# fboehm/DBSLMM

Measured on AMD Instinct MI355X. Metric: SNPs solved/sec (whole node) + max-|Δβ| vs CPU ref, 1M SNP × 10k indiv, higher is better.
Workload: dtype f64

## Files before the change

### dbslmm_amd/csrc/pcg.hip

```cpp
#include <hip/hip_runtime.h>
#include <stdint.h>

namespace pcg {
constexpr int kT = 128;
constexpr int kRunMax = 8;
constexpr int kMaxNC = 4;
constexpr int kWaves = 4;
constexpr int kVS = kT + 8;
constexpr int kNDot = 5;
constexpr int kQS = 8;
constexpr int kThreads = 256;
constexpr int kFTb = 8;
constexpr int kFRows = kFTb * kT;
constexpr int kFPer = kFRows / kThreads;
__device__ __forceinline__ void chip_wide_priority() { __builtin_amdgcn_s_setprio(3); }
constexpr int wave_lds_doubles(int nc) { return 3 * nc * kVS + 4 * nc * 64; }
constexpr size_t lds_bytes(int nc) { return sizeof(double) * kWaves * wave_lds_doubles(nc); }
}

struct PcgBlk {
    int32_t blk, row0, m, ms;
    int32_t ld, Tb, Ns, sco;
    int64_t matoff, vo, po, dof;
    int64_t off16;
    int32_t nc;
    int32_t mshift;
    int32_t fused;
    int32_t pad_;
};

struct PcgArgs {
    const PcgBlk* blk;
    const uint16_t* G16;
    const double* M;
    const int32_t* flags;
    const double* S;
    const double* rsd;
    const double* z;
    const int32_t* slot_out;
    const int32_t* blk_id;
    const double* dshift;
    double *X, *R, *P, *Sv, *W;
    double* U;
    double* part;
    double* dot;
    double* qs;
    int32_t* cnv;
    int32_t* itb;
    int32_t* done;
    int32_t* active;
    int32_t* fin;
    double* beta_s;
    double* beta_l;
    int32_t* status;
    double* mir_s;
    double* mir_l;
    int32_t* mir_st;
    int32_t* mir_flag;
    int32_t run_no;
    int64_t vstride;
    int64_t ns, nl, nbk;
    double tau, rn, c0, tol, inv_sqrt_n;
    int32_t ncopy;
    int32_t run;
    int32_t seed;
};

namespace pcg {

__device__ __forceinline__ void wave_fence() {
    __builtin_amdgcn_fence(__ATOMIC_RELEASE, "wavefront");
    __builtin_amdgcn_wave_barrier();
    __builtin_amdgcn_fence(__ATOMIC_ACQUIRE, "wavefront");
}

template <int Ctrl>
__device__ __forceinline__ double dpp_mov(double v) {
    const uint64_t b = __builtin_bit_cast(uint64_t, v);
    const int lo = __builtin_amdgcn_mov_dpp(static_cast<int>(b & 0xffffffffu), Ctrl, 0xf, 0xf, false);
    const int hi = __builtin_amdgcn_mov_dpp(static_cast<int>(b >> 32), Ctrl, 0xf, 0xf, false);
    return __builtin_bit_cast(double, (static_cast<uint64_t>(static_cast<uint32_t>(hi)) << 32) | static_cast<uint32_t>(lo));
}
template <int X>
__device__ __forceinline__ uint32_t swap_xor(uint32_t x, bool up) {
    if constexpr (X == 16) {
        const auto r = __builtin_amdgcn_permlane16_swap(x, x, false, false);
        return up ? r[0] : r[1];
    } else {
        const auto r = __builtin_amdgcn_permlane32_swap(x, x, false, false);
        return up ? r[0] : r[1];
    }
}
template <int X>
__device__ __forceinline__ double lane_xor(double v) {
#ifndef PCG_NO_DPP
    if constexpr (X == 1) return dpp_mov<0xB1>(v);
    else if constexpr (X == 2) return dpp_mov<0x4E>(v);
    else if constexpr (X == 4) return dpp_mov<0x1B>(dpp_mov<0x141>(v));
    else if constexpr (X == 8) return dpp_mov<0x128>(v);
#ifndef PCG_NO_PERMLANE
    else if constexpr (X == 16 || X == 32) {
        const uint64_t b = __builtin_bit_cast(uint64_t, v);
        const bool up = (__lane_id() & X) != 0;
        const uint32_t lo = swap_xor<X>(static_cast<uint32_t>(b & 0xffffffffu), up);
        const uint32_t hi = swap_xor<X>(static_cast<uint32_t>(b >> 32), up);
        return __builtin_bit_cast(double, (static_cast<uint64_t>(hi) << 32) | lo);
    }
#endif
    else
#endif
        return __shfl_xor(v, X);
}

template <int X2, int X1, int X0>
__device__ __forceinline__ double rscatter8(const double (&v)[8], int lane) {
    const bool h2 = (lane & X2) != 0, h1 = (lane & X1) != 0, h0 = (lane & X0) != 0;
    double u[4], w[2];
#pragma unroll
    for (int q = 0; q < 4; ++q) {
        const double send = h2 ? v[q] : v[q + 4], keep = h2 ? v[q + 4] : v[q];
        u[q] = keep + lane_xor<X2>(send);
    }
#pragma unroll
    for (int q = 0; q < 2; ++q) {
        const double send = h1 ? u[q] : u[q + 2], keep = h1 ? u[q + 2] : u[q];
        w[q] = keep + lane_xor<X1>(send);
    }
    const double send = h0 ? w[0] : w[1], keep = h0 ? w[1] : w[0];
    return keep + lane_xor<X0>(send);
}

__device__ __forceinline__ double wave_sum(double v) {
    v += lane_xor<32>(v);
    v += lane_xor<16>(v);
    v += lane_xor<8>(v);
    v += lane_xor<4>(v);
    v += lane_xor<2>(v);
    v += lane_xor<1>(v);
    return v;
}



__device__ __forceinline__ double ordered_sum(const double* __restrict__ p, int64_t st, int s0, int s1, double acc) {
    for (int s = s0; s < s1; s += 8) {
        double t[8];
#pragma unroll
        for (int u = 0; u < 8; ++u) t[u] = s + u < s1 ? p[static_cast<int64_t>(s + u) * st] : 0.0;
#pragma unroll
        for (int u = 0; u < 8; ++u) acc += t[u];
    }
    return acc;
}

__device__ __forceinline__ bool on_u16(const PcgArgs& a, const PcgBlk& B) {
    return a.G16 != nullptr && (a.flags[B.blk] & 1) == 0;
}

__device__ __forceinline__ double jdiag(const PcgArgs& a, const PcgBlk& B, int i, double dc) {
    return B.mshift ? 1.0 : i < B.ms ? a.c0 + dc : a.c0;
}
__device__ __forceinline__ double col_shift(const PcgArgs& a, const PcgBlk& B, int k) {
    return a.dshift[B.mshift ? a.seed : k];
}

__device__ __forceinline__ void put_beta(const PcgArgs& a, const PcgBlk& B, int i, int k, double x, bool mono) {
    const int so = a.slot_out[B.row0 + i];
    const double bv = mono ? __builtin_nan("") : x * a.inv_sqrt_n;
    if (so >= 0) {
        a.beta_s[k * a.ns + so] = bv;
        if (a.mir_s) a.mir_s[k * a.ns + so] = bv;
    } else {
        a.beta_l[k * a.nl - 1 - so] = bv;
        if (a.mir_l) a.mir_l[k * a.nl - 1 - so] = bv;
    }
}
__device__ __forceinline__ void put_status(const PcgArgs& a, const PcgBlk& B, int k, bool mono) {
    const int st = mono ? DBSLMM_BLOCK_MONOMORPHIC
                        : a.cnv[B.sco + k] == 0 ? DBSLMM_BLOCK_NOT_CONVERGED : DBSLMM_BLOCK_OK;
    const int64_t o = k * a.nbk + a.blk_id[B.blk];
    a.status[o] = st;
    if (a.mir_st) a.mir_st[o] = st;
}

__device__ __forceinline__ double cvt_lo(uint32_t w) {
    double g;
    uint32_t t;
    asm volatile("v_and_b32 %1, 0xffff, %2\n\tv_cvt_f64_u32 %0, %1" : "=v"(g), "=&v"(t) : "v"(w));
    return g;
}
__device__ __forceinline__ double cvt_hi(uint32_t w) {
    double g;
    uint32_t t;
    asm volatile("v_lshrrev_b32 %1, 16, %2\n\tv_cvt_f64_u32 %0, %1" : "=v"(g), "=&v"(t) : "v"(w));
    return g;
}

typedef uint32_t pcg_u4 __attribute__((ext_vector_type(4)));

__device__ __forceinline__ void cvt_row(const pcg_u4& w, double (&g)[8]) {
#pragma unroll
    for (int c = 0; c < 8; ++c) g[c] = (c & 1) ? cvt_hi(w[c >> 1]) : cvt_lo(w[c >> 1]);
}

__device__ __forceinline__ __amdgpu_buffer_rsrc_t g16_rsrc(const uint16_t* base, uint32_t bytes) {
    const uint64_t gb = reinterpret_cast<uint64_t>(base);
    const uint32_t lo = static_cast<uint32_t>(__builtin_amdgcn_readfirstlane(static_cast<int>(gb & 0xffffffffu)));
    const uint32_t hi = static_cast<uint32_t>(__builtin_amdgcn_readfirstlane(static_cast<int>(gb >> 32)));
    const int nb = __builtin_amdgcn_readfirstlane(static_cast<int>(bytes));
    return __builtin_amdgcn_make_buffer_rsrc(reinterpret_cast<void*>((static_cast<uint64_t>(hi) << 32) | lo),
                                             static_cast<short>(0), nb, 0x00020000);
}
constexpr uint32_t kG16Oob = 0x80000000u;

__device__ __forceinline__ void quad_mul16(const pcg_u4 (&raw)[8], bool diagq, int lane, int nc,
                                           const double* vI, const double* vJ, double* rsum, double* csum) {
    const int rg = lane >> 3, cg = lane & 7;
#pragma unroll 1
    for (int k = 0; k < nc; ++k) {
        double vi[8], vj[8], racc[8], cacc[8];
#pragma unroll
        for (int q = 0; q < 8; ++q) {
            vi[q] = vI[k * kVS + 8 * rg + q];
            vj[q] = vJ[k * kVS + 8 * cg + q];
            racc[q] = cacc[q] = 0.0;
        }
        if (!diagq) {
#pragma unroll
            for (int r = 0; r < 8; ++r) {
                double g[8];
                cvt_row(raw[r], g);
#pragma unroll
                for (int c = 0; c < 8; ++c) {
                    racc[r] = __builtin_fma(g[c], vj[c], racc[r]);
                    cacc[c] = __builtin_fma(g[c], vi[r], cacc[c]);
                }
            }
        } else {
#pragma unroll
            for (int r = 0; r < 8; ++r) {
                double g[8];
                cvt_row(raw[r], g);
#pragma unroll
                for (int c = 0; c < 8; ++c) {
                    const int dd = 8 * (cg - rg) + c - r;
                    racc[r] = __builtin_fma(dd <= 0 ? g[c] : 0.0, vj[c], racc[r]);
                    cacc[c] = __builtin_fma(dd < 0 ? g[c] : 0.0, vi[r], cacc[c]);
                }
            }
        }
        rsum[k * 64 + lane] += rscatter8<4, 2, 1>(racc, lane);
        csum[k * 64 + lane] += rscatter8<32, 16, 8>(cacc, lane);
    }
}

__device__ __forceinline__ void quad_mul64(const double* __restrict__ base, int64_t ld, int rows_ok, int cols_ok,
                                           bool diagq, int lane, int nc, const double* vI, const double* vJ,
                                           double* rsum, double* csum) {
    const int rg = lane >> 3, cg = lane & 7;
#pragma unroll 1
    for (int k = 0; k < nc; ++k) {
        double vi[8], vj[8], racc[8], cacc[8];
#pragma unroll
        for (int q = 0; q < 8; ++q) {
            vi[q] = vI[k * kVS + 8 * rg + q];
            vj[q] = vJ[k * kVS + 8 * cg + q];
            racc[q] = cacc[q] = 0.0;
        }
#pragma unroll 1
        for (int r = 0; r < 8; ++r)
#pragma unroll
            for (int c = 0; c < 8; ++c) {
                const double g = (r < rows_ok && c < cols_ok) ? base[r * ld + c] : 0.0;
                const int dd = 8 * (cg - rg) + c - r;
                const double gr = !diagq || dd <= 0 ? g : 0.0, gc = !diagq || dd < 0 ? g : 0.0;
#pragma unroll
                for (int q = 0; q < 8; ++q)
                    if (q == r) racc[q] = __builtin_fma(gr, vj[c], racc[q]);
                cacc[c] = __builtin_fma(gc, vi[r], cacc[c]);
            }
        rsum[k * 64 + lane] += rscatter8<4, 2, 1>(racc, lane);
        csum[k * 64 + lane] += rscatter8<32, 16, 8>(cacc, lane);
    }
}

__device__ __forceinline__ void stage_v(const PcgArgs& a, const PcgBlk& B, int T, int nc, int lane, double* v) {
    for (int k = 0; k < nc; ++k) {
        const double* src = a.U + k * a.vstride + B.vo + static_cast<int64_t>(T) * kT;
        const double x0 = src[lane], x1 = src[lane + 64];
        v[k * kVS + lane] = x0;
        v[k * kVS + lane + 64] = x1;
    }
}

__device__ __forceinline__ bool quad_active(const PcgBlk& B, int I, int J, int q) {
    const int qi = q >> 1, qj = q & 1;
    return !(J == I && qj > qi) && I * kT + 64 * qi < B.m && J * kT + 64 * qj < B.m;
}
__device__ __forceinline__ bool next_quad(const PcgBlk& B, int I, int J1, int& J, int& q) {
    for (;;) {
        if (++q == 4) {
            q = 0;
            if (++J > J1) return false;
        }
        if (quad_active(B, I, J, q)) return true;
    }
}

template <bool U16>
__device__ void symv_item(const PcgArgs& a, int4 item, int lane, double* vI, double* vJb, double* rsum,
                          double* csum) {
    const PcgBlk B = a.blk[item.x];
    if (a.done[item.x] || on_u16(a, B) != U16) return;
    const int I = item.y, J0 = item.z, J1 = item.w, nc = B.nc;
    const int64_t ld16 = static_cast<int64_t>(B.Tb) * kT;
    const int rg = lane >> 3, cg = lane & 7;
    auto vj_of = [&](int J) -> double* { return J == I ? vI : vJb + ((J - J0) & 1) * nc * kVS; };
    const __amdgpu_buffer_rsrc_t g16 =
        g16_rsrc(a.G16 + B.off16 + static_cast<int64_t>(I) * kT * ld16, U16 ? static_cast<uint32_t>(kT * ld16 * 2) : 0u);
    auto load = [&](int J, int q, pcg_u4 (&raw)[8], bool none) {
        if constexpr (U16) {
            const int i0 = 64 * (q >> 1) + 8 * rg, j0 = J * kT + 64 * (q & 1) + 8 * cg;
            const bool skip = none || j0 >= B.m || (J == I && (q == 0 || q == 3) && cg > rg);
            const uint32_t o = static_cast<uint32_t>((static_cast<int64_t>(i0) * ld16 + j0) * 2);
#pragma unroll
            for (int r = 0; r < 8; ++r)
                raw[r] = __builtin_amdgcn_raw_buffer_load_b128(
                    g16, (skip || I * kT + i0 + r >= B.m) ? kG16Oob : o + static_cast<uint32_t>(r * ld16 * 2), 0, 0);
        }
    };
    auto mult = [&](int J, int q, const pcg_u4 (&raw)[8]) {
        const int qi = q >> 1, qj = q & 1;
        const bool dq = J == I && qi == qj;
        const double* vj = vj_of(J);
        double* rs = rsum + qi * nc * 64;
        double* cs = csum + qj * nc * 64;
        if constexpr (U16) {
            quad_mul16(raw, dq, lane, nc, vI + 64 * qi, vj + 64 * qj, rs, cs);
        } else {
            const int ib = I * kT + 64 * qi + 8 * rg, jb = J * kT + 64 * qj + 8 * cg;
            quad_mul64(a.M + B.matoff + static_cast<int64_t>(ib) * B.ld + jb, B.ld, B.m - ib, B.m - jb, dq,
                       lane, nc, vI + 64 * qi, vj + 64 * qj, rs, cs);
        }
    };
    auto flush = [&](int J) {
        double* dst = a.part + B.po + (static_cast<int64_t>(J) * B.Ns + I) * nc * kT;
        for (int qj = 0; qj < 2; ++qj)
            for (int k = 0; k < nc; ++k) {
                dst[k * kT + 64 * qj + 8 * cg + rg] = csum[(qj * nc + k) * 64 + lane];
                csum[(qj * nc + k) * 64 + lane] = 0.0;
            }
    };
    pcg_u4 ra[8], rb[8];
    int J = J0, q = 0;
    load(J, q, ra, false);
    stage_v(a, B, I, nc, lane, vI);
    if (J != I) stage_v(a, B, J, nc, lane, vj_of(J));
    for (int t = 0; t < 2 * nc; ++t) rsum[t * 64 + lane] = csum[t * 64 + lane] = 0.0;
    wave_fence();
    auto step = [&](pcg_u4 (&cur)[8], pcg_u4 (&nxt)[8]) -> bool {
        int Jn = J, qn = q;
        const bool more = next_quad(B, I, J1, Jn, qn);
        load(more ? Jn : J, more ? qn : q, nxt, !more);
        if (more && Jn != J && Jn != I) stage_v(a, B, Jn, nc, lane, vj_of(Jn));
        mult(J, q, cur);
        if (!more || Jn != J) flush(J);
        wave_fence();
        J = Jn;
        q = qn;
        return more;
    };
    while (step(ra, rb) && step(rb, ra)) {
    }
    double* dst = a.part + B.po + (static_cast<int64_t>(I) * B.Ns + B.Tb + J0 / a.run) * nc * kT;
    for (int qi = 0; qi < 2; ++qi)
        for (int k = 0; k < nc; ++k) dst[k * kT + 64 * qi + 8 * rg + cg] = rsum[(qi * nc + k) * 64 + lane];
}

}

extern "C" __global__ __launch_bounds__(pcg::kThreads) void dbslmm_pcg_init(PcgArgs a, const int2* __restrict__ rows,
                                                                            int32_t n_lead, int32_t skip) {
    using namespace pcg;
    __shared__ double red[kThreads / 64][kMaxNC];
    __shared__ int mono_s;
    const int g = blockIdx.x;
    const int2 it = rows[g < n_lead ? g : g + skip];
    const bool head = it.y < 0;
    const int bi = it.x, I = head ? 0 : it.y, tid = threadIdx.x;
    const PcgBlk B = a.blk[bi];
    const bool u16 = on_u16(a, B);
    const int n = a.ncopy, nc = B.nc;
    if (I == 0) {
        if (tid == 0) mono_s = 0;
        __syncthreads();
        bool mono = false;
        for (int i = tid; i < B.m; i += kThreads) mono |= !(a.rsd[B.row0 + i] < INFINITY);
        if (mono) atomicOr(&mono_s, 1);
        __syncthreads();
        if (tid < n) {
            a.cnv[B.sco + tid] = 0;
            double* q = a.qs + static_cast<int64_t>(B.sco + tid) * kQS;
            q[4] = q[5] = 1.0;
        }
        if (tid == 0) {
            a.itb[bi] = 0;
            a.fin[bi] = 0;
            const bool fz = B.fused && u16;
            a.done[bi] = mono_s ? 2 : fz ? 3 : 0;
            if (!mono_s && !fz) atomicAdd(a.active, 1);
        }
    }
    if (head) return;
    const int r = tid & (kT - 1), h = tid >> 7, i = I * kT + r;
    const bool in = i < B.m;
    double sv[kMaxNC];
#pragma unroll
    for (int k = 0; k < kMaxNC; ++k) sv[k] = 0.0;
    for (int c = h; c < n; c += 2) {
        const int64_t o = c * a.vstride + B.vo + i;
        const double rhs = in ? a.z[B.row0 + i] : 0.0;
        a.X[o] = 0.0;
        a.P[o] = 0.0;
        if (c < nc) {
            a.Sv[o] = 0.0;
            a.W[o] = 0.0;
            a.R[o] = rhs;
            double uv = 0.0;
            if (in) {
                uv = rhs / jdiag(a, B, i, col_shift(a, B, c));
                if (u16) uv *= a.rsd[B.row0 + i];
            }
            a.U[o] = uv;
        }
    }
#pragma unroll
    for (int k = 0; k < kMaxNC; ++k)
        if (k < nc && (k & 1) == h && in && u16) {
            const double rhs = a.z[B.row0 + i];
            sv[k] = a.S[B.row0 + i] * a.rsd[B.row0 + i] * (rhs / jdiag(a, B, i, col_shift(a, B, k)));
        }
#pragma unroll
    for (int k = 0; k < kMaxNC; ++k) sv[k] = wave_sum(sv[k]);
    if ((tid & 63) == 0)
#pragma unroll
        for (int k = 0; k < kMaxNC; ++k) red[tid >> 6][k] = sv[k];
    __syncthreads();
    if (tid < nc) {
        const int hk = tid & 1;
        a.dot[B.dof + (static_cast<int64_t>(I) * kNDot + 4) * n + tid] = red[2 * hk][tid] + red[2 * hk + 1][tid];
    }
}

template <bool U16>
__device__ __forceinline__ void symv_body(const PcgArgs& a, const int4* __restrict__ items, int32_t n_items) {
    using namespace pcg;
    extern __shared__ double vlds[];
    chip_wide_priority();
    const int wave = threadIdx.x >> 6, lane = threadIdx.x & 63;
    const int e = blockIdx.x * kWaves + wave;
    if (e >= n_items) return;
    const int nc = a.ncopy;
    double* w = vlds + wave * wave_lds_doubles(nc);
    symv_item<U16>(a, items[e], lane, w, w + nc * kVS, w + 3 * nc * kVS, w + 3 * nc * kVS + 2 * nc * 64);
}
#ifndef PCG_SYMV_WAVES
#define PCG_SYMV_WAVES 2
#endif
extern "C" __global__ __launch_bounds__(pcg::kThreads) __attribute__((amdgpu_waves_per_eu(PCG_SYMV_WAVES, 8)))
void dbslmm_pcg_symv16(PcgArgs a, const int4* __restrict__ items, int32_t n_items) {
    symv_body<true>(a, items, n_items);
}
extern "C" __global__ __launch_bounds__(pcg::kThreads)
void dbslmm_pcg_symv64(PcgArgs a, const int4* __restrict__ items, int32_t n_items) {
    symv_body<false>(a, items, n_items);
}

extern "C" __global__ __launch_bounds__(pcg::kThreads) void dbslmm_pcg_rows(PcgArgs a, const int2* __restrict__ rows) {
    using namespace pcg;
    __shared__ double red[kThreads / 64][kMaxNC][4];
    __shared__ double sig[kMaxNC];
    chip_wide_priority();
    const int2 it = rows[blockIdx.x];
    const int bi = it.x, I = it.y, tid = threadIdx.x;
    if (a.done[bi]) return;
    const PcgBlk B = a.blk[bi];
    const bool u16 = on_u16(a, B);
    const int n = a.ncopy, nc = B.nc;
    if (tid < nc)
        sig[tid] = ordered_sum(a.dot + B.dof + 4 * n + tid, kNDot * n, 0, B.Tb, 0.0);
    __syncthreads();
    const int r = tid & (kT - 1), h = tid >> 7, i = I * kT + r;
    const bool in = i < B.m;
    const double Si = in ? a.S[B.row0 + i] : 0.0, ri = in ? a.rsd[B.row0 + i] : 0.0;
    const int nrun = (I + a.run) / a.run;
    double dv[kMaxNC][4];
#pragma unroll
    for (int k = 0; k < kMaxNC; ++k)
#pragma unroll
        for (int f = 0; f < 4; ++f) dv[k][f] = 0.0;
#pragma unroll
    for (int k = 0; k < kMaxNC; ++k) {
        if (k >= n || (k & 1) != h) continue;
        const int64_t o = k * a.vstride + B.vo + i;
        if (k < nc) {
            const double* pp = a.part + B.po + static_cast<int64_t>(I) * B.Ns * nc * kT + k * kT + r;
            double y = ordered_sum(pp, nc * kT, I, B.Tb, 0.0);
            y = ordered_sum(pp, nc * kT, B.Tb, B.Tb + nrun, y);
            const double dc = col_shift(a, B, k);
            const double rv = a.R[o];
            const double u = in ? rv / jdiag(a, B, i, dc) : 0.0;
            const double sh = i < B.ms ? dc : 0.0;
            double w = 0.0;
            if (in) {
                if (u16) w = a.tau * a.rn * ri * __builtin_fma(-Si, sig[k] * a.rn, y) + (1.0 - a.tau + sh) * u;
                else w = y + sh * u;
            }
            a.W[o] = w;
            dv[k][0] = rv * u;
            dv[k][1] = w * u;
            dv[k][2] = rv * rv;
        }
        const double xv = a.X[o];
        dv[k][3] = xv * xv;
    }
#pragma unroll
    for (int k = 0; k < kMaxNC; ++k)
#pragma unroll
        for (int f = 0; f < 4; ++f) dv[k][f] = wave_sum(dv[k][f]);
    if ((tid & 63) == 0)
#pragma unroll
        for (int k = 0; k < kMaxNC; ++k)
#pragma unroll
            for (int f = 0; f < 4; ++f) red[tid >> 6][k][f] = dv[k][f];
    __syncthreads();
    if (tid < 4 * n) {
        const int k = tid >> 2, f = tid & 3, hk = k & 1;
        if (f == 3 || k < nc)
            a.dot[B.dof + (static_cast<int64_t>(I) * kNDot + f) * n + k] = red[2 * hk][k][f] + red[2 * hk + 1][k][f];
    }
    if (I == 0 && tid == 0) a.itb[bi] += 1;
}

extern "C" __global__ __launch_bounds__(pcg::kThreads) void dbslmm_pcg_update(PcgArgs a, const int2* __restrict__ rows) {
    using namespace pcg;
    __shared__ double tot[kMaxNC][4];
    __shared__ double coef[kMaxNC][3];
    __shared__ double seedc[2];
    __shared__ int run_s[kMaxNC];
    __shared__ double red[kThreads / 64][kMaxNC];
    chip_wide_priority();
    const int2 it = rows[blockIdx.x];
    const int bi = it.x, I = it.y, tid = threadIdx.x;
    if (a.done[bi]) return;
    const PcgBlk B = a.blk[bi];
    const bool u16 = on_u16(a, B);
    const int n = a.ncopy, nc = B.nc;
    const int itn = a.itb[bi] - 1;
    const int par = itn & 1;
    if (tid < 4 * n) {
        const int k = tid >> 2, f = tid & 3;
        tot[k][f] = (f == 3 || k < nc) ? ordered_sum(a.dot + B.dof + f * n + k, kNDot * n, 0, B.Tb, 0.0) : 0.0;
    }
    __syncthreads();
    if (B.mshift) {
        if (tid == 0) {
            const double gam = tot[0][0], del = tot[0][1];
            const double* q = a.qs + static_cast<int64_t>(B.sco) * kQS;
            double al, be = 0.0;
            if (itn == 0) {
                al = gam / del;
            } else {
                be = gam / q[2 * par];
                al = gam / (del - be * gam / q[2 * par + 1]);
            }
            seedc[0] = al;
            seedc[1] = be;
        }
        __syncthreads();
        if (tid < n) {
            const int c = tid;
            double* q = a.qs + static_cast<int64_t>(B.sco + c) * kQS;
            const double al = seedc[0], be = seedc[1];
            const double zk = q[4 + 2 * par], zk1 = q[4 + 2 * par + 1];
            const double rr = tot[0][2] * zk * zk, xx = tot[c][3];
            const double t = a.tol * (a.dshift[c] + 1.0 - a.tau);
            const bool conv = a.cnv[B.sco + c] != 0 || rr == 0.0 || rr <= t * t * xx;
            const double e = a.dshift[c] - a.dshift[a.seed];
            const double cp = itn == 0 ? 0.0 : al * be / a.qs[static_cast<int64_t>(B.sco) * kQS + 2 * par + 1];
            const double zn = zk * zk1 / ((1.0 + cp + al * e) * zk1 - cp * zk);
            coef[c][0] = al * zn / zk;
            coef[c][1] = zk1 != 0.0 ? (zk / zk1) * (zk / zk1) * be : 0.0;
            coef[c][2] = zk;
            run_s[c] = conv ? 0 : 1;
            if (I == 0) {
                if (conv && a.cnv[B.sco + c] == 0) a.cnv[B.sco + c] = itn + 1;
                q[4 + 2 * (par ^ 1)] = zn;
                q[4 + 2 * (par ^ 1) + 1] = zk;
            }
        }
        __syncthreads();
        if (I == 0 && tid == 0) {
            double* q = a.qs + static_cast<int64_t>(B.sco) * kQS;
            q[2 * (par ^ 1)] = tot[0][0];
            q[2 * (par ^ 1) + 1] = seedc[0];
        }
    } else {
        if (tid < n) {
            const int k = tid;
            const double gam = tot[k][0], del = tot[k][1], rr = tot[k][2], xx = tot[k][3];
            const double lam = B.ms == B.m ? a.dshift[k] + 1.0 - a.tau : 1.0 - a.tau;
            const double t = a.tol * lam;
            const bool conv = a.cnv[B.sco + k] != 0 || rr == 0.0 || rr <= t * t * xx;
            double al = 0.0, be = 0.0;
            if (!conv) {
                double* q = a.qs + static_cast<int64_t>(B.sco + k) * kQS;
                if (itn == 0) {
                    al = gam / del;
                } else {
                    be = gam / q[2 * par];
                    al = gam / (del - be * gam / q[2 * par + 1]);
                }
                if (I == 0) {
                    q[2 * (par ^ 1)] = gam;
                    q[2 * (par ^ 1) + 1] = al;
                }
            } else if (I == 0 && a.cnv[B.sco + k] == 0) {
                a.cnv[B.sco + k] = itn + 1;
            }
            coef[k][0] = al;
            coef[k][1] = be;
            coef[k][2] = 1.0;
            run_s[k] = conv ? 0 : 1;
        }
        __syncthreads();
    }
    int running = 0;
    for (int k = 0; k < n; ++k) running += run_s[k];
    if (running == 0) {
        const int r = tid & (kT - 1), h = tid >> 7, i = I * kT + r;
        if (i < B.m)
            for (int k = h; k < n; k += 2) put_beta(a, B, i, k, a.X[k * a.vstride + B.vo + i], false);
        if (I == 0 && tid < n) put_status(a, B, tid, false);
        __syncthreads();
        if (tid == 0 &&
            __hip_atomic_fetch_add(a.fin + bi, 1, __ATOMIC_ACQ_REL, __HIP_MEMORY_SCOPE_AGENT) == B.Tb - 1) {
            a.done[bi] = 1;
            atomicSub(a.active, 1);
            if (a.mir_flag)
                for (int c = 0; c < n; ++c)
                    __hip_atomic_store(a.mir_flag + static_cast<int64_t>(bi) * n + c, a.run_no, __ATOMIC_RELEASE,
                                       __HIP_MEMORY_SCOPE_SYSTEM);
        }
        return;
    }
    const int r = tid & (kT - 1), h = tid >> 7, i = I * kT + r;
    const bool in = i < B.m;
    double sv[kMaxNC];
#pragma unroll
    for (int k = 0; k < kMaxNC; ++k) sv[k] = 0.0;
    if (B.mshift) {
        if (in) {
            const int64_t o0 = B.vo + i;
            const double rv = a.R[o0];
#pragma unroll
            for (int c = 0; c < kMaxNC; ++c) {
                if (c >= n || (c & 1) != h || !run_s[c]) continue;
                const int64_t o = c * a.vstride + o0;
                const double p = __builtin_fma(coef[c][1], a.P[o], coef[c][2] * rv);
                a.P[o] = p;
                a.X[o] = __builtin_fma(coef[c][0], p, a.X[o]);
            }
            if (h == 0) {
                const double al = seedc[0], be = seedc[1];
                const double sn = __builtin_fma(be, a.Sv[o0], a.W[o0]);
                const double rn = __builtin_fma(-al, sn, rv);
                a.Sv[o0] = sn;
                a.R[o0] = rn;
                a.U[o0] = u16 ? rn * a.rsd[B.row0 + i] : rn;
                if (u16) sv[0] = a.S[B.row0 + i] * a.rsd[B.row0 + i] * rn;
            }
        }
    } else {
#pragma unroll
        for (int k = 0; k < kMaxNC; ++k) {
            if (k >= n || (k & 1) != h || !run_s[k] || !in) continue;
            const int64_t o = k * a.vstride + B.vo + i;
            const double al = coef[k][0], be = coef[k][1];
            const double dg = jdiag(a, B, i, a.dshift[k]);
            const double u = a.R[o] / dg;
            const double p = __builtin_fma(be, a.P[o], u);
            const double s = __builtin_fma(be, a.Sv[o], a.W[o]);
            const double x = __builtin_fma(al, p, a.X[o]);
            const double rn = __builtin_fma(-al, s, a.R[o]);
            a.P[o] = p;
            a.Sv[o] = s;
            a.X[o] = x;
            a.R[o] = rn;
            a.U[o] = u16 ? (rn / dg) * a.rsd[B.row0 + i] : rn / dg;
            if (u16) sv[k] = a.S[B.row0 + i] * a.rsd[B.row0 + i] * (rn / dg);
        }
    }
#pragma unroll
    for (int k = 0; k < kMaxNC; ++k) sv[k] = wave_sum(sv[k]);
    if ((tid & 63) == 0)
#pragma unroll
        for (int k = 0; k < kMaxNC; ++k) red[tid >> 6][k] = sv[k];
    __syncthreads();
    if (tid < nc && (B.mshift || run_s[tid])) {
        const int hk = tid & 1;
        a.dot[B.dof + (static_cast<int64_t>(I) * kNDot + 4) * n + tid] = red[2 * hk][tid] + red[2 * hk + 1][tid];
    }
}

namespace pcg {
template <int N>
__device__ __forceinline__ void block_sum(double (&v)[N], double* red, int tid) {
#pragma unroll
    for (int k = 0; k < N; ++k) v[k] = wave_sum(v[k]);
    __syncthreads();
    if ((tid & 63) == 0)
#pragma unroll
        for (int k = 0; k < N; ++k) red[(tid >> 6) * N + k] = v[k];
    __syncthreads();
#pragma unroll
    for (int k = 0; k < N; ++k) v[k] = ((red[k] + red[N + k]) + red[2 * N + k]) + red[3 * N + k];
}
constexpr size_t block_lds_bytes(int n) {
    return sizeof(double) * ((5 + 2 * n) * kFRows + 4 * (3 + kMaxNC) + 12 + 3 * kMaxNC + 4);
}
}

__device__ __forceinline__ void pcg_block_solve(const PcgArgs& a, int bi, int cc, int32_t maxit) {
    using namespace pcg;
    extern __shared__ double blds[];
    double* yw = blds;
    double* Ul = blds + 4 * kFRows;
    const int n = a.ncopy;
    double* Xl = Ul + kFRows;
    double* Pl = Xl + n * kFRows;
    double* red = Pl + n * kFRows;
    if (a.done[bi] != 3) return;
    const PcgBlk B = a.blk[bi];
    const int tid = threadIdx.x, lane = tid & 63;
    const int wave = __builtin_amdgcn_readfirstlane(tid >> 6);
    const int m = B.m, Tb = B.Tb;
    const bool msh = cc < 0;
    const int nx = msh ? n : 1;
    const double dc = msh ? col_shift(a, B, 0) : a.dshift[cc];
    const int Q = (m + 63) / 64;
    const int nq = Q * (Q + 1) / 2;
    const int nw = (nq + 3 - wave) >> 2;
    const int64_t ld16 = static_cast<int64_t>(Tb) * kT;
    const int rg = lane >> 3, cg = lane & 7;
    struct QPos {
        int t, qi, qj;
    };
    auto adv = [](QPos& p, int k) {
        p.t += k;
        p.qj += k;
        while (p.qj > p.qi) {
            p.qj -= p.qi + 1;
            ++p.qi;
        }
    };
    QPos first{0, 0, 0};
    adv(first, wave);
    QPos second = first;
    adv(second, 4);
    const __amdgpu_buffer_rsrc_t g16 = g16_rsrc(a.G16 + B.off16, static_cast<uint32_t>(ld16 * ld16 * 2));
    auto load = [&](const QPos& p, pcg_u4 (&raw)[8]) {
        const int r0 = 64 * p.qi + 8 * rg, c0 = 64 * p.qj + 8 * cg;
        const bool skip = p.t >= nq || c0 >= m || (p.qi == p.qj && cg > rg);
        const uint32_t o = static_cast<uint32_t>((r0 * static_cast<int>(ld16) + c0) * 2);
#pragma unroll
        for (int rr = 0; rr < 8; ++rr)
            raw[rr] = __builtin_amdgcn_raw_buffer_load_b128(
                g16, (skip || r0 + rr >= m) ? kG16Oob : o + static_cast<uint32_t>(rr * ld16 * 2), 0, 0);
    };
    pcg_u4 ra[8], rb[8], rc[8];
    load(first, ra);
    load(second, rb);
    double r[kFPer], sv[kFPer], wv[kFPer], Sr[kFPer], Rr[kFPer], sg[1] = {0.0};
#pragma unroll
    for (int q = 0; q < kFPer; ++q) {
        const int i = tid + kThreads * q;
        const bool in = i < m;
        r[q] = in ? a.z[B.row0 + i] : 0.0;
        Sr[q] = in ? a.S[B.row0 + i] : 0.0;
        Rr[q] = in ? a.rsd[B.row0 + i] : 0.0;
        sv[q] = wv[q] = 0.0;
        double u = 0.0;
        if (in) {
            u = (r[q] / jdiag(a, B, i, dc)) * Rr[q];
            sg[0] += Sr[q] * u;
        }
        Ul[i] = u;
        for (int w = 0; w < 4; ++w) yw[w * kFRows + i] = 0.0;
        for (int c = 0; c < nx; ++c) Xl[c * kFRows + i] = Pl[c * kFRows + i] = 0.0;
    }
    block_sum(sg, red, tid);
    double sig = sg[0];
    auto mult = [&](const QPos& p, const pcg_u4 (&raw)[8]) {
        const int qi = p.qi, qj = p.qj;
        const bool dq = qi == qj;
        double vi[8], vj[8], racc[8], cacc[8];
#pragma unroll
        for (int q = 0; q < 8; ++q) {
            vi[q] = Ul[64 * qi + 8 * rg + q];
            vj[q] = Ul[64 * qj + 8 * cg + q];
            racc[q] = cacc[q] = 0.0;
        }
        if (!dq) {
#pragma unroll
            for (int rr = 0; rr < 8; ++rr) {
                double g[8];
                cvt_row(raw[rr], g);
#pragma unroll
                for (int c = 0; c < 8; ++c) {
                    racc[rr] = __builtin_fma(g[c], vj[c], racc[rr]);
                    cacc[c] = __builtin_fma(g[c], vi[rr], cacc[c]);
                }
            }
        } else {
#pragma unroll
            for (int rr = 0; rr < 8; ++rr) {
                double g[8];
                cvt_row(raw[rr], g);
#pragma unroll
                for (int c = 0; c < 8; ++c) {
                    const int dd = 8 * (cg - rg) + c - rr;
                    racc[rr] = __builtin_fma(dd <= 0 ? g[c] : 0.0, vj[c], racc[rr]);
                    cacc[c] = __builtin_fma(dd < 0 ? g[c] : 0.0, vi[rr], cacc[c]);
                }
            }
        }
        double* y = yw + wave * kFRows;
        const int ri = 64 * qi + 8 * rg + cg, ci = 64 * qj + 8 * cg + rg;
        y[ri] += rscatter8<4, 2, 1>(racc, lane);
        wave_fence();
        y[ci] += rscatter8<32, 16, 8>(cacc, lane);
    };
    double* st = red + 4 * (3 + kMaxNC);
    int* flag = reinterpret_cast<int*>(st + 12 + 3 * kMaxNC);
    if (tid == 0) {
        for (int c = 0; c < kMaxNC; ++c) {
            st[4 + c] = st[8 + c] = 1.0;
            flag[c] = c >= n;
        }
    }
    int it = 0;
    for (; it < maxit; ++it) {
        __syncthreads();
        {
            QPos pm = first, pl = second;
            adv(pl, 4);
            int s = 0;
            for (; s + 3 < nw; s += 3) {
                load(pl, rc);
                adv(pl, 4);
                mult(pm, ra);
                adv(pm, 4);
                load(pl, ra);
                adv(pl, 4);
                mult(pm, rb);
                adv(pm, 4);
                load(pl, rb);
                adv(pl, 4);
                mult(pm, rc);
                adv(pm, 4);
            }
            if (nw > 0) {
                const int rem = nw - s;
                load(pl, rc);
                mult(pm, ra);
                adv(pm, 4);
                load(first, ra);
                if (rem >= 2) {
                    mult(pm, rb);
                    adv(pm, 4);
                }
                load(second, rb);
                if (rem >= 3) mult(pm, rc);
            }
        }
        __syncthreads();
        double d[3 + kMaxNC];
#pragma unroll
        for (int k = 0; k < 3 + kMaxNC; ++k) d[k] = 0.0;
#pragma unroll
        for (int q = 0; q < kFPer; ++q) {
            const int i = tid + kThreads * q;
            double y = 0.0;
            if (i < Tb * kT) {
                y = ((yw[i] + yw[kFRows + i]) + yw[2 * kFRows + i]) + yw[3 * kFRows + i];
#pragma unroll
                for (int w = 0; w < 4; ++w) yw[w * kFRows + i] = 0.0;
            }
            if (i < m) {
                const double Si = Sr[q], ri = Rr[q];
                const double u = r[q] / jdiag(a, B, i, dc);
                const double sh = i < B.ms ? dc : 0.0;
                const double w = a.tau * a.rn * ri * __builtin_fma(-Si, sig * a.rn, y) + (1.0 - a.tau + sh) * u;
                wv[q] = w;
                d[0] += r[q] * u;
                d[1] += w * u;
                d[2] += r[q] * r[q];
                for (int c = 0; c < nx; ++c) {
                    const double xv = Xl[c * kFRows + i];
                    d[3 + c] += xv * xv;
                }
            }
        }
        block_sum(d, red, tid);
        if (tid == 0) {
            const double gam = d[0], del = d[1], rr = d[2];
            double al, be = 0.0;
            if (it == 0) {
                al = gam / del;
            } else {
                be = gam / st[0];
                al = gam / (del - be * gam / st[1]);
            }
            int running = 0;
            if (msh) {
                const double cp = it == 0 ? 0.0 : al * be / st[1];
                for (int c = 0; c < n; ++c) {
                    const double zk = st[4 + c], zk1 = st[8 + c];
                    const double t = a.tol * (a.dshift[c] + 1.0 - a.tau);
                    const double rrc = rr * zk * zk;
                    if (!flag[c] && (rrc == 0.0 || rrc <= t * t * d[3 + c])) {
                        flag[c] = 1;
                        a.cnv[B.sco + c] = it + 1;
                    }
                    const double e = a.dshift[c] - a.dshift[a.seed];
                    const double zn = zk * zk1 / ((1.0 + cp + al * e) * zk1 - cp * zk);
                    st[12 + 3 * c] = al * zn / zk;
                    st[12 + 3 * c + 1] = zk1 != 0.0 ? (zk / zk1) * (zk / zk1) * be : 0.0;
                    st[12 + 3 * c + 2] = zk;
                    st[8 + c] = zk;
                    st[4 + c] = zn;
                    running += flag[c] ? 0 : 1;
                }
            } else {
                const double lam = B.ms == B.m ? dc + 1.0 - a.tau : 1.0 - a.tau;
                const double t = a.tol * lam;
                if (rr == 0.0 || rr <= t * t * d[3]) {
                    flag[0] = 1;
                    a.cnv[B.sco + cc] = it + 1;
                }
                running = flag[0] ? 0 : 1;
            }
            st[0] = gam;
            st[1] = al;
            st[2] = al;
            st[3] = be;
            flag[kMaxNC] = running;
        }
        __syncthreads();
        if (flag[kMaxNC] == 0) break;
        const double al = st[2], be = st[3];
        double sg2[1] = {0.0};
#pragma unroll
        for (int q = 0; q < kFPer; ++q) {
            const int i = tid + kThreads * q;
            if (i >= m) continue;
            const double rsd_i = Rr[q];
            double rn;
            if (msh) {
                for (int c = 0; c < n; ++c) {
                    if (flag[c]) continue;
                    const int o = c * kFRows + i;
                    const double pv = __builtin_fma(st[12 + 3 * c + 1], Pl[o], st[12 + 3 * c + 2] * r[q]);
                    Pl[o] = pv;
                    Xl[o] = __builtin_fma(st[12 + 3 * c], pv, Xl[o]);
                }
                const double sn = __builtin_fma(be, sv[q], wv[q]);
                rn = __builtin_fma(-al, sn, r[q]);
                sv[q] = sn;
                r[q] = rn;
                Ul[i] = rn * rsd_i;
            } else {
                const double dg = jdiag(a, B, i, dc);
                const double u = r[q] / dg;
                const double pv = __builtin_fma(be, Pl[i], u);
                const double sn = __builtin_fma(be, sv[q], wv[q]);
                Pl[i] = pv;
                Xl[i] = __builtin_fma(al, pv, Xl[i]);
                rn = __builtin_fma(-al, sn, r[q]);
                sv[q] = sn;
                r[q] = rn;
                Ul[i] = (rn / dg) * rsd_i;
            }
            sg2[0] += Sr[q] * Ul[i];
        }
        block_sum(sg2, red, tid);
        sig = sg2[0];
    }
#pragma unroll
    for (int q = 0; q < kFPer; ++q) {
        const int i = tid + kThreads * q;
        if (i < m)
            for (int c = 0; c < nx; ++c) put_beta(a, B, i, msh ? c : cc, Xl[c * kFRows + i], false);
    }
    if (tid == 0) {
        atomicMax(a.itb + bi, it + (it < maxit ? 1 : 0));
        for (int c = 0; c < nx; ++c) put_status(a, B, msh ? c : cc, false);
    }
    if (a.mir_flag) {
        __syncthreads();
        if (tid == 0)
            for (int c = 0; c < nx; ++c)
                __hip_atomic_store(a.mir_flag + static_cast<int64_t>(bi) * n + (msh ? c : cc), a.run_no,
                                   __ATOMIC_RELEASE, __HIP_MEMORY_SCOPE_SYSTEM);
    }
}

extern "C" __global__ __launch_bounds__(pcg::kThreads)
__attribute__((amdgpu_waves_per_eu(1, 8), amdgpu_num_vgpr(312)))
void dbslmm_pcg_block(PcgArgs a, const int2* __restrict__ list, int32_t n_list, int32_t* __restrict__ next,
                      int32_t maxit) {
    __shared__ int e_s;
    for (;;) {
        __syncthreads();
        if (threadIdx.x == 0) e_s = atomicAdd(next, 1);
        __syncthreads();
        const int e = e_s;
        if (e >= n_list) break;
        pcg_block_solve(a, list[e].x, list[e].y, maxit);
    }
}

extern "C" __global__ __launch_bounds__(pcg::kThreads) void dbslmm_pcg_final(PcgArgs a, const int2* __restrict__ rows) {
    using namespace pcg;
    const int2 it = rows[blockIdx.x];
    const int bi = it.x, I = it.y, tid = threadIdx.x;
    const int done = a.done[bi];
    if (done == 3 || done == 1) return;
    const PcgBlk B = a.blk[bi];
    const bool mono = done == 2;
    const int r = tid & (kT - 1), h = tid >> 7, i = I * kT + r;
    if (i < B.m)
        for (int k = h; k < a.ncopy; k += 2) put_beta(a, B, i, k, a.X[k * a.vstride + B.vo + i], mono);
    if (I == 0 && tid < a.ncopy) put_status(a, B, tid, mono);
}
```

Measured before the change: 164.5 million.

## Retile u16 SYMV quads to 16x4 lane tiles with row-accumulator reuse and contiguous wave ranges

Changes each lane's micro-tile in the 64x64 u16 quad kernels from 8x8 to 16 rows by 4 columns, loaded with b64 buffer loads. Row accumulators and the vi vector now stay in registers across consecutive quads that share a row block, so the row reduction and store happen only when the row block ends. The fused block solver deals quads to waves as contiguous ranges rather than round-robin, which is what allows that reuse. Diagonal handling now masks the strictly-upper part with bit operations and adds the diagonal term separately through an extra b16 load or a preloaded Gd. This removes per-element select logic and repeated row reductions, at the cost of more register pressure and new diagonal and flush bookkeeping that could cause errors.

```diff
diff --git a/dbslmm_amd/csrc/pcg.hip b/dbslmm_amd/csrc/pcg.hip
--- a/dbslmm_amd/csrc/pcg.hip
+++ b/dbslmm_amd/csrc/pcg.hip
@@ -1,5 +1,7 @@
 #include <hip/hip_runtime.h>
 #include <stdint.h>
+
+#include "pcg_deal.hpp"
 
 namespace pcg {
 constexpr int kT = 128;
@@ -93,23 +95,32 @@
 }
 template <int X>
 __device__ __forceinline__ double lane_xor(double v) {
-#ifndef PCG_NO_DPP
+    static_assert(X == 1 || X == 2 || X == 4 || X == 8 || X == 16 || X == 32, "one lane bit");
     if constexpr (X == 1) return dpp_mov<0xB1>(v);
     else if constexpr (X == 2) return dpp_mov<0x4E>(v);
     else if constexpr (X == 4) return dpp_mov<0x1B>(dpp_mov<0x141>(v));
     else if constexpr (X == 8) return dpp_mov<0x128>(v);
-#ifndef PCG_NO_PERMLANE
-    else if constexpr (X == 16 || X == 32) {
+    else {
         const uint64_t b = __builtin_bit_cast(uint64_t, v);
         const bool up = (__lane_id() & X) != 0;
         const uint32_t lo = swap_xor<X>(static_cast<uint32_t>(b & 0xffffffffu), up);
         const uint32_t hi = swap_xor<X>(static_cast<uint32_t>(b >> 32), up);
         return __builtin_bit_cast(double, (static_cast<uint64_t>(hi) << 32) | lo);
     }
-#endif
-    else
-#endif
-        return __shfl_xor(v, X);
+}
+
+template <int N, int X, int... Xs>
+__device__ __forceinline__ double rscatter(const double (&v)[N], int lane) {
+    static_assert(N == (2 << sizeof...(Xs)), "one lane bit per halving");
+    const bool h = (lane & X) != 0;
+    double u[N / 2];
+#pragma unroll
+    for (int q = 0; q < N / 2; ++q) {
+        const double send = h ? v[q] : v[q + N / 2], keep = h ? v[q + N / 2] : v[q];
+        u[q] = keep + lane_xor<X>(send);
+    }
+    if constexpr (sizeof...(Xs) == 0) return u[0];
+    else return rscatter<N / 2, Xs...>(u, lane);
 }
 
 template <int X2, int X1, int X0>
@@ -196,11 +207,11 @@
     return g;
 }
 
-typedef uint32_t pcg_u4 __attribute__((ext_vector_type(4)));
-
-__device__ __forceinline__ void cvt_row(const pcg_u4& w, double (&g)[8]) {
-#pragma unroll
-    for (int c = 0; c < 8; ++c) g[c] = (c & 1) ? cvt_hi(w[c >> 1]) : cvt_lo(w[c >> 1]);
+typedef uint32_t pcg_u2 __attribute__((ext_vector_type(2)));
+
+__device__ __forceinline__ void cvt_row(const pcg_u2& w, double (&g)[4]) {
+#pragma unroll
+    for (int c = 0; c < 4; ++c) g[c] = (c & 1) ? cvt_hi(w[c >> 1]) : cvt_lo(w[c >> 1]);
 }
 
 __device__ __forceinline__ __amdgpu_buffer_rsrc_t g16_rsrc(const uint16_t* base, uint32_t bytes) {
@@ -213,44 +224,62 @@
 }
 constexpr uint32_t kG16Oob = 0x80000000u;
 
-__device__ __forceinline__ void quad_mul16(const pcg_u4 (&raw)[8], bool diagq, int lane, int nc,
-                                           const double* vI, const double* vJ, double* rsum, double* csum) {
-    const int rg = lane >> 3, cg = lane & 7;
+constexpr int kQRows = 16, kQCols = 4;
+__device__ __forceinline__ void quad_strict(pcg_u2 (&raw)[kQRows], int dbase) {
+#pragma unroll
+    for (int r = 0; r < kQRows; ++r) {
+        const int keep = r - dbase;
+        raw[r].x = keep >= 2 ? raw[r].x : keep == 1 ? raw[r].x & 0xffffu : 0u;
+        raw[r].y = keep >= 4 ? raw[r].y : keep == 3 ? raw[r].y & 0xffffu : 0u;
+    }
+}
+__device__ __forceinline__ void quad_fma(const pcg_u2 (&raw)[kQRows], const double (&vi)[kQRows],
+                                         const double (&vj)[kQCols], double (&racc)[kQRows], double (&cacc)[kQCols]) {
+#pragma unroll
+    for (int r = 0; r < kQRows; ++r) {
+        double g[kQCols];
+        cvt_row(raw[r], g);
+#pragma unroll
+        for (int c = 0; c < kQCols; ++c) {
+            racc[r] = __builtin_fma(g[c], vj[c], racc[r]);
+            cacc[c] = __builtin_fma(g[c], vi[r], cacc[c]);
+        }
+    }
+}
+__device__ __forceinline__ double col_sum(const double (&cacc)[kQCols], int lane) {
+    return rscatter<kQCols, 32, 16>(cacc, lane);
+}
+__device__ __forceinline__ double row_sum(const double (&racc)[kQRows], int lane) {
+    return rscatter<kQRows, 8, 4, 2, 1>(racc, lane);
+}
+
+__device__ __forceinline__ void quad_mul16(pcg_u2 (&raw)[kQRows], uint32_t gd, bool diagq, int lane, int nc, bool fresh,
+                                           bool last, const double* vI, const double* vJ, double* rsum, double* csum,
+                                           double (&vi)[kQRows], double (&racc)[kQRows]) {
+    const int rg = lane >> 4, cg = lane & 15;
+    if (diagq) quad_strict(raw, kQCols * cg - kQRows * rg);
 #pragma unroll 1
     for (int k = 0; k < nc; ++k) {
-        double vi[8], vj[8], racc[8], cacc[8];
-#pragma unroll
-        for (int q = 0; q < 8; ++q) {
-            vi[q] = vI[k * kVS + 8 * rg + q];
-            vj[q] = vJ[k * kVS + 8 * cg + q];
-            racc[q] = cacc[q] = 0.0;
-        }
-        if (!diagq) {
-#pragma unroll
-            for (int r = 0; r < 8; ++r) {
-                double g[8];
-                cvt_row(raw[r], g);
-#pragma unroll
-                for (int c = 0; c < 8; ++c) {
-                    racc[r] = __builtin_fma(g[c], vj[c], racc[r]);
-                    cacc[c] = __builtin_fma(g[c], vi[r], cacc[c]);
-                }
-            }
-        } else {
-#pragma unroll
-            for (int r = 0; r < 8; ++r) {
-                double g[8];
-                cvt_row(raw[r], g);
-#pragma unroll
-                for (int c = 0; c < 8; ++c) {
-                    const int dd = 8 * (cg - rg) + c - r;
-                    racc[r] = __builtin_fma(dd <= 0 ? g[c] : 0.0, vj[c], racc[r]);
-                    cacc[c] = __builtin_fma(dd < 0 ? g[c] : 0.0, vi[r], cacc[c]);
-                }
-            }
-        }
-        rsum[k * 64 + lane] += rscatter8<4, 2, 1>(racc, lane);
-        csum[k * 64 + lane] += rscatter8<32, 16, 8>(cacc, lane);
+        double vj[kQCols], cacc[kQCols];
+        if (fresh) {
+#pragma unroll
+            for (int q = 0; q < kQRows; ++q) {
+                vi[q] = vI[k * kVS + kQRows * rg + q];
+                racc[q] = 0.0;
+            }
+        }
+#pragma unroll
+        for (int q = 0; q < kQCols; ++q) {
+            vj[q] = vJ[k * kVS + kQCols * cg + q];
+            cacc[q] = 0.0;
+        }
+        quad_fma(raw, vi, vj, racc, cacc);
+        csum[k * 64 + lane] += col_sum(cacc, lane);
+        if (last) {
+            double rs = row_sum(racc, lane);
+            if (diagq) rs = __builtin_fma(cvt_lo(gd), vI[k * kVS + lane], rs);
+            rsum[k * 64 + lane] += rs;
+        }
     }
 }
 
@@ -314,29 +343,40 @@
     if (a.done[item.x] || on_u16(a, B) != U16) return;
     const int I = item.y, J0 = item.z, J1 = item.w, nc = B.nc;
     const int64_t ld16 = static_cast<int64_t>(B.Tb) * kT;
-    const int rg = lane >> 3, cg = lane & 7;
+    const int rg = U16 ? lane >> 4 : lane >> 3, cg = U16 ? lane & 15 : lane & 7;
+    const int rrow = U16 ? lane : 8 * rg + cg, rcol = U16 ? kQCols * cg + rg : 8 * cg + rg;
     auto vj_of = [&](int J) -> double* { return J == I ? vI : vJb + ((J - J0) & 1) * nc * kVS; };
+    const int rows_in = B.m - I * kT < kT ? B.m - I * kT : kT;
     const __amdgpu_buffer_rsrc_t g16 =
-        g16_rsrc(a.G16 + B.off16 + static_cast<int64_t>(I) * kT * ld16, U16 ? static_cast<uint32_t>(kT * ld16 * 2) : 0u);
-    auto load = [&](int J, int q, pcg_u4 (&raw)[8], bool none) {
+        g16_rsrc(a.G16 + B.off16 + static_cast<int64_t>(I) * kT * ld16, U16 ? static_cast<uint32_t>(rows_in * ld16 * 2) : 0u);
+    const int rstride = __builtin_amdgcn_readfirstlane(static_cast<int>(ld16) * 2);
+    auto load = [&](int J, int q, pcg_u2 (&raw)[kQRows], uint32_t& gd, bool none) {
         if constexpr (U16) {
-            const int i0 = 64 * (q >> 1) + 8 * rg, j0 = J * kT + 64 * (q & 1) + 8 * cg;
-            const bool skip = none || j0 >= B.m || (J == I && (q == 0 || q == 3) && cg > rg);
-            const uint32_t o = static_cast<uint32_t>((static_cast<int64_t>(i0) * ld16 + j0) * 2);
-#pragma unroll
-            for (int r = 0; r < 8; ++r)
-                raw[r] = __builtin_amdgcn_raw_buffer_load_b128(
-                    g16, (skip || I * kT + i0 + r >= B.m) ? kG16Oob : o + static_cast<uint32_t>(r * ld16 * 2), 0, 0);
+            const int i0 = 64 * (q >> 1) + kQRows * rg, j0 = J * kT + 64 * (q & 1) + kQCols * cg;
+            const bool skip = none || j0 >= B.m ||
+                              (J == I && (q == 0 || q == 3) && kQCols * cg > kQRows * rg + kQRows - 1);
+            const uint32_t o = skip ? kG16Oob : static_cast<uint32_t>((static_cast<int64_t>(i0) * ld16 + j0) * 2);
+#pragma unroll
+            for (int r = 0; r < kQRows; ++r)
+                raw[r] = __builtin_amdgcn_raw_buffer_load_b64(g16, o, r * rstride, 0);
+            const int il = 64 * (q >> 1) + lane;
+            const bool dg = !none && J == I && (q == 0 || q == 3);
+            gd = __builtin_amdgcn_raw_buffer_load_b16(
+                g16, dg ? static_cast<uint32_t>((static_cast<int64_t>(il) * ld16 + J * kT + il) * 2) : kG16Oob, 0, 0);
         }
     };
-    auto mult = [&](int J, int q, const pcg_u4 (&raw)[8]) {
+    double vi[kQRows], racc[kQRows];
+    bool fresh = true;
+    auto mult = [&](int J, int q, pcg_u2 (&raw)[kQRows], uint32_t gd, bool same_rows_next) {
         const int qi = q >> 1, qj = q & 1;
         const bool dq = J == I && qi == qj;
         const double* vj = vj_of(J);
         double* rs = rsum + qi * nc * 64;
         double* cs = csum + qj * nc * 64;
         if constexpr (U16) {
-            quad_mul16(raw, dq, lane, nc, vI + 64 * qi, vj + 64 * qj, rs, cs);
+            const bool last = nc > 1 || !same_rows_next || dq;
+            quad_mul16(raw, gd, dq, lane, nc, fresh, last, vI + 64 * qi, vj + 64 * qj, rs, cs, vi, racc);
+            fresh = last;
         } else {
             const int ib = I * kT + 64 * qi + 8 * rg, jb = J * kT + 64 * qj + 8 * cg;
             quad_mul64(a.M + B.matoff + static_cast<int64_t>(ib) * B.ld + jb, B.ld, B.m - ib, B.m - jb, dq,
@@ -347,34 +387,35 @@
         double* dst = a.part + B.po + (static_cast<int64_t>(J) * B.Ns + I) * nc * kT;
         for (int qj = 0; qj < 2; ++qj)
             for (int k = 0; k < nc; ++k) {
-                dst[k * kT + 64 * qj + 8 * cg + rg] = csum[(qj * nc + k) * 64 + lane];
+                dst[k * kT + 64 * qj + rcol] = csum[(qj * nc + k) * 64 + lane];
                 csum[(qj * nc + k) * 64 + lane] = 0.0;
             }
     };
-    pcg_u4 ra[8], rb[8];
+    pcg_u2 ra[kQRows], rb[kQRows];
+    uint32_t ga = 0, gb = 0;
     int J = J0, q = 0;
-    load(J, q, ra, false);
+    load(J, q, ra, ga, false);
     stage_v(a, B, I, nc, lane, vI);
     if (J != I) stage_v(a, B, J, nc, lane, vj_of(J));
     for (int t = 0; t < 2 * nc; ++t) rsum[t * 64 + lane] = csum[t * 64 + lane] = 0.0;
     wave_fence();
-    auto step = [&](pcg_u4 (&cur)[8], pcg_u4 (&nxt)[8]) -> bool {
+    auto step = [&](pcg_u2 (&cur)[kQRows], uint32_t gcur, pcg_u2 (&nxt)[kQRows], uint32_t& gnxt) -> bool {
         int Jn = J, qn = q;
         const bool more = next_quad(B, I, J1, Jn, qn);
-        load(more ? Jn : J, more ? qn : q, nxt, !more);
+        load(more ? Jn : J, more ? qn : q, nxt, gnxt, !more);
         if (more && Jn != J && Jn != I) stage_v(a, B, Jn, nc, lane, vj_of(Jn));
-        mult(J, q, cur);
+        mult(J, q, cur, gcur, more && Jn == J && (qn >> 1) == (q >> 1));
         if (!more || Jn != J) flush(J);
         wave_fence();
         J = Jn;
         q = qn;
         return more;
     };
-    while (step(ra, rb) && step(rb, ra)) {
+    while (step(ra, ga, rb, gb) && step(rb, gb, ra, ga)) {
     }
     double* dst = a.part + B.po + (static_cast<int64_t>(I) * B.Ns + B.Tb + J0 / a.run) * nc * kT;
     for (int qi = 0; qi < 2; ++qi)
-        for (int k = 0; k < nc; ++k) dst[k * kT + 64 * qi + 8 * rg + cg] = rsum[(qi * nc + k) * 64 + lane];
+        for (int k = 0; k < nc; ++k) dst[k * kT + 64 * qi + rrow] = rsum[(qi * nc + k) * 64 + lane];
 }
 
 }
@@ -464,10 +505,7 @@
     double* w = vlds + wave * wave_lds_doubles(nc);
     symv_item<U16>(a, items[e], lane, w, w + nc * kVS, w + 3 * nc * kVS, w + 3 * nc * kVS + 2 * nc * 64);
 }
-#ifndef PCG_SYMV_WAVES
-#define PCG_SYMV_WAVES 2
-#endif
-extern "C" __global__ __launch_bounds__(pcg::kThreads) __attribute__((amdgpu_waves_per_eu(PCG_SYMV_WAVES, 8)))
+extern "C" __global__ __launch_bounds__(pcg::kThreads) __attribute__((amdgpu_waves_per_eu(2, 8)))
 void dbslmm_pcg_symv16(PcgArgs a, const int4* __restrict__ items, int32_t n_items) {
     symv_body<true>(a, items, n_items);
 }
@@ -748,40 +786,30 @@
     const bool msh = cc < 0;
     const int nx = msh ? n : 1;
     const double dc = msh ? col_shift(a, B, 0) : a.dshift[cc];
+    using pcg_deal::QPos;
     const int Q = (m + 63) / 64;
-    const int nq = Q * (Q + 1) / 2;
-    const int nw = (nq + 3 - wave) >> 2;
+    const int nq = pcg_deal::num_quads(Q);
+    const int t0 = pcg_deal::range_begin(nq, wave), t1 = pcg_deal::range_end(nq, wave);
+    const int nw = t1 - t0;
     const int64_t ld16 = static_cast<int64_t>(Tb) * kT;
-    const int rg = lane >> 3, cg = lane & 7;
-    struct QPos {
-        int t, qi, qj;
+    const int rg = lane >> 4, cg = lane & 15;
+    const QPos first = pcg_deal::pos_of(t0);
+    QPos second = first;
+    pcg_deal::advance(second);
+    const __amdgpu_buffer_rsrc_t g16 = g16_rsrc(a.G16 + B.off16, static_cast<uint32_t>(m * ld16 * 2));
+    const int rstride = static_cast<int>(ld16) * 2;
+    auto load = [&](const QPos& p, pcg_u2 (&raw)[kQRows]) {
+        const int r0 = 64 * p.qi + kQRows * rg, c0 = 64 * p.qj + kQCols * cg;
+        const bool skip = p.t >= t1 || c0 >= m || (p.qi == p.qj && kQCols * cg > kQRows * rg + kQRows - 1);
+        const uint32_t o = skip ? kG16Oob : static_cast<uint32_t>((r0 * static_cast<int>(ld16) + c0) * 2);
+#pragma unroll
+        for (int rr = 0; rr < kQRows; ++rr)
+            raw[rr] = __builtin_amdgcn_raw_buffer_load_b64(g16, o, rr * rstride, 0);
     };
-    auto adv = [](QPos& p, int k) {
-        p.t += k;
-        p.qj += k;
-        while (p.qj > p.qi) {
-            p.qj -= p.qi + 1;
-            ++p.qi;
-        }
-    };
-    QPos first{0, 0, 0};
-    adv(first, wave);
-    QPos second = first;
-    adv(second, 4);
-    const __amdgpu_buffer_rsrc_t g16 = g16_rsrc(a.G16 + B.off16, static_cast<uint32_t>(ld16 * ld16 * 2));
-    auto load = [&](const QPos& p, pcg_u4 (&raw)[8]) {
-        const int r0 = 64 * p.qi + 8 * rg, c0 = 64 * p.qj + 8 * cg;
-        const bool skip = p.t >= nq || c0 >= m || (p.qi == p.qj && cg > rg);
-        const uint32_t o = static_cast<uint32_t>((r0 * static_cast<int>(ld16) + c0) * 2);
-#pragma unroll
-        for (int rr = 0; rr < 8; ++rr)
-            raw[rr] = __builtin_amdgcn_raw_buffer_load_b128(
-                g16, (skip || r0 + rr >= m) ? kG16Oob : o + static_cast<uint32_t>(rr * ld16 * 2), 0, 0);
-    };
-    pcg_u4 ra[8], rb[8], rc[8];
+    pcg_u2 ra[kQRows], rb[kQRows], rc[kQRows];
     load(first, ra);
     load(second, rb);
-    double r[kFPer], sv[kFPer], wv[kFPer], Sr[kFPer], Rr[kFPer], sg[1] = {0.0};
+    double r[kFPer], sv[kFPer], wv[kFPer], Sr[kFPer], Rr[kFPer], Gd[kFPer], sg[1] = {0.0};
 #pragma unroll
     for (int q = 0; q < kFPer; ++q) {
         const int i = tid + kThreads * q;
@@ -789,6 +817,7 @@
         r[q] = in ? a.z[B.row0 + i] : 0.0;
         Sr[q] = in ? a.S[B.row0 + i] : 0.0;
         Rr[q] = in ? a.rsd[B.row0 + i] : 0.0;
+        Gd[q] = in ? static_cast<double>(a.G16[B.off16 + i * ld16 + i]) : 0.0;
         sv[q] = wv[q] = 0.0;
         double u = 0.0;
         if (in) {
@@ -801,45 +830,33 @@
     }
     block_sum(sg, red, tid);
     double sig = sg[0];
-    auto mult = [&](const QPos& p, const pcg_u4 (&raw)[8]) {
+    double vi[kQRows], racc[kQRows];
+#pragma unroll
+    for (int q = 0; q < kQRows; ++q) racc[q] = 0.0;
+    auto load_vi = [&](int qi) {
+#pragma unroll
+        for (int q = 0; q < kQRows; ++q) vi[q] = Ul[64 * qi + kQRows * rg + q];
+    };
+    auto mult = [&](const QPos& p, pcg_u2 (&raw)[kQRows]) {
         const int qi = p.qi, qj = p.qj;
-        const bool dq = qi == qj;
-        double vi[8], vj[8], racc[8], cacc[8];
-#pragma unroll
-        for (int q = 0; q < 8; ++q) {
-            vi[q] = Ul[64 * qi + 8 * rg + q];
-            vj[q] = Ul[64 * qj + 8 * cg + q];
-            racc[q] = cacc[q] = 0.0;
-        }
-        if (!dq) {
-#pragma unroll
-            for (int rr = 0; rr < 8; ++rr) {
-                double g[8];
-                cvt_row(raw[rr], g);
-#pragma unroll
-                for (int c = 0; c < 8; ++c) {
-                    racc[rr] = __builtin_fma(g[c], vj[c], racc[rr]);
-                    cacc[c] = __builtin_fma(g[c], vi[rr], cacc[c]);
-                }
-            }
-        } else {
-#pragma unroll
-            for (int rr = 0; rr < 8; ++rr) {
-                double g[8];
-                cvt_row(raw[rr], g);
-#pragma unroll
-                for (int c = 0; c < 8; ++c) {
-                    const int dd = 8 * (cg - rg) + c - rr;
-                    racc[rr] = __builtin_fma(dd <= 0 ? g[c] : 0.0, vj[c], racc[rr]);
-                    cacc[c] = __builtin_fma(dd < 0 ? g[c] : 0.0, vi[rr], cacc[c]);
-                }
-            }
-        }
+        double vj[kQCols], cacc[kQCols];
+#pragma unroll
+        for (int q = 0; q < kQCols; ++q) {
+            vj[q] = Ul[64 * qj + kQCols * cg + q];
+            cacc[q] = 0.0;
+        }
+        if (qi == qj) quad_strict(raw, kQCols * cg - kQRows * rg);
+        quad_fma(raw, vi, vj, racc, cacc);
         double* y = yw + wave * kFRows;
-        const int ri = 64 * qi + 8 * rg + cg, ci = 64 * qj + 8 * cg + rg;
-        y[ri] += rscatter8<4, 2, 1>(racc, lane);
-        wave_fence();
-        y[ci] += rscatter8<32, 16, 8>(cacc, lane);
+        y[64 * qj + kQCols * cg + rg] += col_sum(cacc, lane);
+        if (pcg_deal::flush_after(p, t1)) {
+            wave_fence();
+            y[64 * qi + lane] += row_sum(racc, lane);
+#pragma unroll
+            for (int q = 0; q < kQRows; ++q) racc[q] = 0.0;
+            wave_fence();
+            if (p.t + 1 < t1) load_vi(qi + 1);
+        }
     };
     double* st = red + 4 * (3 + kMaxNC);
     int* flag = reinterpret_cast<int*>(st + 12 + 3 * kMaxNC);
@@ -853,32 +870,34 @@
     for (; it < maxit; ++it) {
         __syncthreads();
         {
+            using pcg_deal::advance;
             QPos pm = first, pl = second;
-            adv(pl, 4);
+            advance(pl);
+            if (nw > 0) load_vi(first.qi);
             int s = 0;
             for (; s + 3 < nw; s += 3) {
                 load(pl, rc);
-                adv(pl, 4);
+                advance(pl);
                 mult(pm, ra);
-                adv(pm, 4);
+                advance(pm);
                 load(pl, ra);
-                adv(pl, 4);
+                advance(pl);
                 mult(pm, rb);
-                adv(pm, 4);
+                advance(pm);
                 load(pl, rb);
-                adv(pl, 4);
+                advance(pl);
                 mult(pm, rc);
-                adv(pm, 4);
+                advance(pm);
             }
             if (nw > 0) {
                 const int rem = nw - s;
                 load(pl, rc);
                 mult(pm, ra);
-                adv(pm, 4);
+                advance(pm);
                 load(first, ra);
                 if (rem >= 2) {
                     mult(pm, rb);
-                    adv(pm, 4);
+                    advance(pm);
                 }
                 load(second, rb);
                 if (rem >= 3) mult(pm, rc);
@@ -898,6 +917,7 @@
                 for (int w = 0; w < 4; ++w) yw[w * kFRows + i] = 0.0;
             }
             if (i < m) {
+                y = __builtin_fma(Gd[q], Ul[i], y);
                 const double Si = Sr[q], ri = Rr[q];
                 const double u = r[q] / jdiag(a, B, i, dc);
                 const double sh = i < B.ms ? dc : 0.0;
@@ -958,7 +978,7 @@
             flag[kMaxNC] = running;
         }
         __syncthreads();
-        if (flag[kMaxNC] == 0) break;
+        if (__builtin_amdgcn_readfirstlane(flag[kMaxNC]) == 0) break;
         const double al = st[2], be = st[3];
         double sg2[1] = {0.0};
 #pragma unroll
@@ -1025,7 +1045,7 @@
         __syncthreads();
         if (threadIdx.x == 0) e_s = atomicAdd(next, 1);
         __syncthreads();
-        const int e = e_s;
+        const int e = __builtin_amdgcn_readfirstlane(e_s);
         if (e >= n_list) break;
         pcg_block_solve(a, list[e].x, list[e].y, maxit);
     }
diff --git a/dbslmm_amd/csrc/pcg_deal.hpp b/dbslmm_amd/csrc/pcg_deal.hpp
--- /dev/null
+++ b/dbslmm_amd/csrc/pcg_deal.hpp
@@ -0,0 +1,36 @@
+#pragma once
+
+namespace pcg_deal {
+
+constexpr int kWaves = 4;
+
+struct QPos {
+    int t, qi, qj;
+};
+
+constexpr int num_quads(int Q) { return Q * (Q + 1) / 2; }
+constexpr int range_begin(int nq, int w) { return w * nq / kWaves; }
+constexpr int range_end(int nq, int w) { return (w + 1) * nq / kWaves; }
+
+constexpr QPos pos_of(int t) {
+    QPos p{t, 0, t};
+    while (p.qj > p.qi) {
+        p.qj -= p.qi + 1;
+        ++p.qi;
+    }
+    return p;
+}
+
+constexpr void advance(QPos& p) {
+    ++p.t;
+    if (p.qj == p.qi) {
+        ++p.qi;
+        p.qj = 0;
+    } else {
+        ++p.qj;
+    }
+}
+
+constexpr bool flush_after(const QPos& p, int end) { return p.qj == p.qi || p.t + 1 >= end; }
+
+}
```

New measurement: 163.9 million. Within noise of the previous version (-0.4%).
